# FraPria/proovread

Hardware: AMD Instinct MI355X
Metric: corrected long-read Mbases/sec per node (higher is better)
Workload: dtype int32

## Files before the change

proovread_amd/csrc/seed_core.h:

```cpp
#pragma once
#include <math.h>
#include <stdint.h>

#include "../../include/prgpu.h"

#if defined(__HIPCC__)
#define SC_HD __host__ __device__ inline
#else
#define SC_HD inline
#endif

#if defined(PR_SEED_STATS) && !defined(__HIP_DEVICE_COMPILE__)
extern unsigned long long pr_seed_stat_g[24];
#define SC_STAT(k, v) __atomic_fetch_add(&pr_seed_stat_g[k], (unsigned long long)(v), __ATOMIC_RELAXED)
#else
#define SC_STAT(k, v) ((void)0)
#endif

namespace prgpu {
namespace seedc {

constexpr int KI = 12;
constexpr uint32_t NK = 1u << (2 * KI);
constexpr int KX = 28;
constexpr uint64_t KX_MASK = (1ull << (2 * KX)) - 1;
#ifndef SC_SCANGE
#define SC_SCANGE 1
#endif
constexpr int HB = 20;
constexpr int CB_SHIFT = 12;
constexpr int RK = 11;

constexpr uint64_t POS_PAGE = 1ull << 32;
constexpr int64_t MAX_TEXT = (int64_t)1 << 33;

struct BlkFr {
    int64_t d0, d1;
    int32_t c0, bnd, bnd2, pad;
};

struct IndexView {
    const uint8_t *text;
    int64_t n_text;
    const int64_t *cstart;
    int32_t n_contig;
    const int32_t *cblk;
    const int64_t *lr_off;
    int32_t n_lr;
    int64_t l_pac;
    const uint64_t *koff;
    const uint32_t *kpos;
    const uint64_t *ksplit;
    const uint64_t *kext;
    const uint32_t *cnt[KI - 1];
    const uint64_t *text4;
    const BlkFr *blkfr;
    int32_t walk_nw = 4;
};

struct Iv {
    int32_t start, end;
    int64_t occ;
};
struct Seed {
    int64_t rbeg;
    int16_t qbeg, len;
    int32_t nx;
};
struct RangeRec {
    int32_t head, tail, n, l_idx;
    int64_t tpos;
    int64_t f_rbeg, l_rbeg;
    int32_t f_ql, l_ql;
    int32_t pad[4];
};
struct RangeEnt {
    int32_t key, r;
};
struct Chain {
    int64_t pos;
    int32_t rid, head, tail, n;
    int32_t w, kept, first;
};

enum {
    SC_OVER_LEN = 1, SC_OVER_HITS = 2, SC_OVER_IV = 4, SC_OVER_MEMS = 8, SC_OVER_SEEDS = 16,
    SC_OVER_CHAINS = 32, SC_OVER_OUT = 64
};

struct Scratch {
    int32_t lmax;
    int32_t *hoff;
    uint64_t *qext;
    int32_t *codes;
    uint32_t *ge;
    uint32_t *hpos;
    uint8_t *hhi;
    uint16_t *hml;
    int32_t cap_hits;
    Iv *mems;
    int32_t cap_mems;
    Iv *m1, *curr, *prev;
    int32_t cap_iv;
    Seed *seeds;
    int32_t cap_seeds;
    Chain *cv, *ch;
    int32_t *cnx, *kept;
    RangeEnt *htab;
    RangeRec *rg;
    int32_t cap_chains, hsize;
    uint16_t *rmax;
    uint64_t *hfr;
    int32_t *hend;
    uint8_t *ready;
    uint64_t *q4w;
    int32_t *lz;
    int32_t lim_hits;
    bool htab_clean;
};

SC_HD uint64_t pack_ext(const uint8_t *s, int n) {
    uint64_t v = 0;
    int k = 0;
    for (; k < n && s[k] < 4; ++k) v |= (uint64_t)s[k] << (2 * k);
    return v | ((uint64_t)k << 56);
}

SC_HD int ctz64(uint64_t x) { return __builtin_ctzll(x); }

SC_HD uint8_t base_code(uint8_t c) {
    if (c < 4) return c;
    switch (c | 0x20) {
        case 'a': return 0;
        case 'c': return 1;
        case 'g': return 2;
        case 't': return 3;
        default: return 4;
    }
}

SC_HD uint64_t hit_pos(const IndexView &I, uint32_t code, uint64_t r) {
    uint64_t p = I.kpos[r];
    if (I.ksplit && r >= I.ksplit[code]) p += POS_PAGE;
    return p;
}
SC_HD uint64_t get_hpos(const Scratch &S, int64_t k) {
    return (uint64_t)S.hpos[k] | (S.hhi ? (uint64_t)S.hhi[k] << 32 : 0ull);
}
SC_HD void set_hpos(const Scratch &S, int64_t k, uint64_t p) {
    if (!S.hpos) return;
    S.hpos[k] = (uint32_t)p;
    if (S.hhi) S.hhi[k] = (uint8_t)(p >> 32);
}

SC_HD int contig_of(const IndexView &I, int64_t p) {
    int c = I.cblk[p >> CB_SHIFT];
    while (c + 1 < I.n_contig && I.cstart[c + 1] <= p) ++c;
    return c;
}

SC_HD void text_to_fr(const IndexView &I, uint64_t p, int64_t &fr, int &rid) {
    const int c = contig_of(I, p);
    const int64_t o = (int64_t)p - I.cstart[c];
    if (c < I.n_lr) {
        rid = c;
        fr = I.lr_off[c] + o;
// ... 567 lines not shown
        if constexpr (occ_lazy<OccT>::value) return S.lz[1] != 0;
        else return false;
    };
    auto push = [&](const Iv &v) {
        if (nm >= S.cap_mems) {
            err |= SC_OVER_MEMS;
            return;
        }
        S.mems[nm++] = v;
    };
    for (int x = 0; x < len && !err && !over();) {
        if (q[x] < 4) {
            x = smem1(occ, S, q, len, x, 1, S.m1, n1, err);
            for (int k = 0; k < n1; ++k)
                if (S.m1[k].end - S.m1[k].start >= O.min_seed_len) push(S.m1[k]);
        } else {
            ++x;
        }
    }
    SC_TICK(0);
    const int split_len = (int)(O.min_seed_len * O.split_factor + .499);
    const int nfirst = nm;
    for (int k = 0; k < nfirst && !err && !over(); ++k) {
        const Iv p = S.mems[k];
        if (p.end - p.start < split_len || p.occ > O.split_width) continue;
        smem1(occ, S, q, len, (p.start + p.end) >> 1, p.occ + 1, S.m1, n1, err);
        for (int j = 0; j < n1; ++j)
            if (S.m1[j].end - S.m1[j].start >= O.min_seed_len) push(S.m1[j]);
    }
    SC_TICK(1);
    if (O.max_mem_intv > 0) {
        for (int x = 0; x < len && !err && !over();) {
            if (q[x] < 4) {
                Iv m;
                x = seed_strategy1(occ, q, len, x, O.min_seed_len, O.max_mem_intv, m);
                if (m.occ > 0) push(m);
            } else {
                ++x;
            }
        }
    }
    if (over()) return nm;
    if (nm > 1 && S.cap_seeds >= nm && !err && !S.hend) {
        static_assert(sizeof(Seed) == sizeof(Iv), "the seed pool holds the sorted intervals");
        int32_t *cnt = S.codes;
        Iv *tmp = reinterpret_cast<Iv *>(S.seeds);
        for (int x = 0; x <= len; ++x) cnt[x] = 0;
        for (int i = 0; i < nm; ++i) ++cnt[S.mems[i].start + 1];
        for (int x = 1; x <= len; ++x) cnt[x] += cnt[x - 1];
        for (int i = 0; i < nm; ++i) {
            const Iv v = S.mems[i];
            tmp[cnt[v.start]++] = v;
        }
        for (int i = 0; i < nm; ++i) {
            const Iv v = tmp[i];
            int j = i - 1;
            while (j >= 0 && S.mems[j].start == v.start && S.mems[j].end > v.end) {
                S.mems[j + 1] = S.mems[j];
                --j;
            }
            S.mems[j + 1] = v;
        }
    } else {
        for (int i = 1; i < nm; ++i) {
            const Iv v = S.mems[i];
            int j = i - 1;
            while (j >= 0 && (S.mems[j].start > v.start || (S.mems[j].start == v.start && S.mems[j].end > v.end))) {
                S.mems[j + 1] = S.mems[j];
                --j;
            }
            S.mems[j + 1] = v;
        }
    }
    SC_TICK(2);
    return nm;
}

SC_HD int range_slot(const Scratch &S, int32_t key) {
    uint32_t h = ((uint32_t)key * 0x9E3779B1u) & (uint32_t)(S.hsize - 1);
    while (S.htab[h].key != -1 && S.htab[h].key != key) h = (h + 1) & (uint32_t)(S.hsize - 1);
    return (int)h;
}
SC_HD int32_t pack_ql(const Seed &s) { return (int32_t)(uint16_t)s.qbeg | ((int32_t)s.len << 16); }

SC_HD int test_and_merge(const pr_seed_opts &O, int64_t l_pac, Scratch &S, int32_t &ns, Chain &c, const Seed &p,
                         int rid) {
    const Seed &last = S.seeds[c.tail];
    const Seed &first = S.seeds[c.head];
    const int64_t qend = last.qbeg + last.len, rend = last.rbeg + last.len;
    if (rid != c.rid) return 0;
    if (p.qbeg >= first.qbeg && p.qbeg + p.len <= qend && p.rbeg >= first.rbeg && p.rbeg + p.len <= rend)
        return 1;
    if ((last.rbeg < l_pac || first.rbeg < l_pac) && p.rbeg >= l_pac) return 0;
    const int64_t x = p.qbeg - last.qbeg, y = p.rbeg - last.rbeg;
    if (y >= 0 && x - y <= O.w && y - x <= O.w && x - last.len < O.max_chain_gap && y - last.len < O.max_chain_gap) {
        if (ns >= S.cap_seeds) return -1;
        S.seeds[ns] = p;
        S.seeds[ns].nx = -1;
        S.seeds[c.tail].nx = ns;
        c.tail = ns++;
        ++c.n;
        return 1;
    }
    return 0;
}

SC_HD int merge_tail(const pr_seed_opts &O, int64_t l_pac, Scratch &S, int32_t &ns, RangeRec &R, const Seed &p) {
    const int64_t f_rbeg = R.f_rbeg, l_rbeg = R.l_rbeg;
    const int f_q = (int16_t)(R.f_ql & 0xFFFF), l_q = (int16_t)(R.l_ql & 0xFFFF), l_len = R.l_ql >> 16;
    const int64_t qend = l_q + l_len, rend = l_rbeg + l_len;
    if (p.qbeg >= f_q && p.qbeg + p.len <= qend && p.rbeg >= f_rbeg && p.rbeg + p.len <= rend)
        return 1;
    if ((l_rbeg < l_pac || f_rbeg < l_pac) && p.rbeg >= l_pac) return 0;
    const int64_t x = p.qbeg - l_q, y = p.rbeg - l_rbeg;
    if (y >= 0 && x - y <= O.w && y - x <= O.w && x - l_len < O.max_chain_gap && y - l_len < O.max_chain_gap) {
        if (ns >= S.cap_seeds) return -1;
        S.seeds[ns] = p;
        S.seeds[ns].nx = -1;
        S.seeds[R.l_idx].nx = ns;
        R.l_idx = ns++;
        R.l_rbeg = p.rbeg;
        R.l_ql = pack_ql(p);
        ++R.n;
        return 1;
    }
    return 0;
}
SC_HD void flush_tail(Scratch &S, const RangeRec &R) {
    S.cv[R.tail].tail = R.l_idx;
    S.cv[R.tail].n = R.n;
}

SC_HD int chain_weight(const Scratch &S, const Chain &c) {
    int64_t qe = 0, re = 0;
    int wq = 0, wr = 0;
    for (int32_t k = c.head; k >= 0;) {
        const Seed s = S.seeds[k];
        if (s.qbeg >= qe) wq += s.len;
        else if (s.qbeg + s.len > qe) wq += (int)(s.qbeg + s.len - qe);
        qe = qe > s.qbeg + s.len ? qe : s.qbeg + s.len;
        if (s.rbeg >= re) wr += s.len;
        else if (s.rbeg + s.len > re) wr += (int)(s.rbeg + s.len - re);
        re = re > s.rbeg + s.len ? re : s.rbeg + s.len;
        k = s.nx;
    }
    const int w = wr < wq ? wr : wq;
    return w < (1 << 30) ? w : (1 << 30) - 1;
}

SC_HD int cal_max_gap(const pr_seed_opts &O, int qlen) {
    int l_del = (int)((double)(qlen * O.a - O.o_del) / O.e_del + 1.);
    int l_ins = (int)((double)(qlen * O.a - O.o_ins) / O.e_ins + 1.);
    int l = l_del > l_ins ? l_del : l_ins;
    l = l > 1 ? l : 1;
    return l < O.w << 1 ? l : O.w << 1;
}

SC_HD int seed_flt_min_score(const pr_seed_opts &O, int len) {
    double min_l;
    if (O.min_chain_weight) min_l = (double)(1.1f * (float)O.min_chain_weight);
    else min_l = (double)5.5f * log((double)len);
    if (min_l > (double)(0.05f * (float)len)) return -1;
    return (int)(O.a * min_l + .499);
}

template <class T>
SC_HD int seed_sw_score(const IndexView &I, const pr_seed_opts &O, const uint8_t *q, int len, const Seed &s, int rid,
                        T *H, T *E, int stride = 1) {
    if (s.len >= 200) return -1;
    int qb = s.qbeg - 50, qe = s.qbeg + s.len + 50;
    qb = qb > 0 ? qb : 0;
    qe = qe < len ? qe : len;
    int64_t rb = s.rbeg - 50, re = s.rbeg + s.len + 50;
    const int64_t mid = (s.rbeg + s.rbeg + s.len) >> 1;
    rb = rb > 0 ? rb : 0;
    re = re < (I.l_pac << 1) ? re : (I.l_pac << 1);
    if (rb < I.l_pac && I.l_pac < re) {
        if (mid < I.l_pac) re = I.l_pac;
        else rb = I.l_pac;
    }
    if (qe - qb >= 200 || re - rb >= 200) return -1;
    const bool rev = mid >= I.l_pac;
    const int64_t fb = rev ? (I.l_pac << 1) - I.lr_off[rid + 1] : I.lr_off[rid];
    const int64_t fe = rev ? (I.l_pac << 1) - I.lr_off[rid] : I.lr_off[rid + 1];
    rb = rb > fb ? rb : fb;
    re = re < fe ? re : fe;
    const int64_t tc = rev ? I.cstart[2 * I.n_lr - 1 - rid] : I.cstart[rid];
    const uint8_t *t = I.text + tc + (rb - fb);
    const int qn = qe - qb, tn = (int)(re - rb);
    const int oe_del = O.o_del + O.e_del, oe_ins = O.o_ins + O.e_ins;
    for (int j = 0; j < qn; ++j) H[j * stride] = 0, E[j * stride] = 0;
    int best = 0;
    for (int i = 0; i < tn; ++i) {
        const int ti = t[i];
        int hdiag = 0, f = 0;
        for (int j = 0; j < qn; ++j) {
            const int qj = q[qb + j];
            const int sc = (ti > 3 || qj > 3) ? -1 : (ti == qj ? O.a : -O.b);
            int h = hdiag + sc;
            const int e = E[j * stride];
            h = h > e ? h : e;
            h = h > f ? h : f;
            h = h > 0 ? h : 0;
            hdiag = H[j * stride];
            H[j * stride] = (T)h;
            best = best > h ? best : h;
            int en = e - O.e_del, eo = h - oe_del;
            en = en > eo ? en : eo;
            E[j * stride] = (T)(en > 0 ? en : 0);
            int fn = f - O.e_ins, fo = h - oe_ins;
            fn = fn > fo ? fn : fo;
            f = fn > 0 ? fn : 0;
        }
    }
    return best;
}

SC_HD void chain_flt(const pr_seed_opts &O, Scratch &S, int ncv, int *n_chains);
template <bool LZ = false>
SC_HD int chain_seq(const IndexView &I, const pr_seed_opts &O, Scratch &S, int nm, int *n_cv);

template <bool LZ = false>
SC_HD int map_chains(const IndexView &I, const pr_seed_opts &O, Scratch &S, const uint8_t *q, int len, int *n_chains,
                     unsigned long long *ticks = nullptr, const uint32_t *lcnt = nullptr) {
    *n_chains = 0;
    int err = 0;
#if defined(__HIP_DEVICE_COMPILE__)
    unsigned long long t_last = ticks ? __builtin_amdgcn_s_memrealtime() : 0ULL;
#endif
    const OccB<LZ> occ{&I, &S, q, len, lcnt};
    const int nm = collect_intv(occ, S, O, q, len, err, ticks);
    if (LZ) err |= S.lz[1];
    if (err) return err;
    SC_STAT(0, 1);
    SC_STAT(1, nm);
#if defined(__HIP_DEVICE_COMPILE__)
    if (ticks) t_last = __builtin_amdgcn_s_memrealtime();
#endif
    int ncv = 0;
    err = chain_seq<LZ>(I, O, S, nm, &ncv);
    if (LZ) err |= S.lz[1];
    if (err) return err;
    SC_TICK(3);
    SC_STAT(11, ncv);
    SC_STAT(12, (unsigned long long)ncv * ncv);
    chain_flt(O, S, ncv, n_chains);
    SC_TICK(4);
    return 0;
}

template <bool LZ>
SC_HD int chain_seq(const IndexView &I, const pr_seed_opts &O, Scratch &S, int nm, int *n_cv) {
    const bool clean_on_entry = S.htab_clean;
    int32_t ns = 0, ncv = 0, nrg = 0;
    if (!clean_on_entry)
        for (int k = 0; k < S.hsize; ++k) S.htab[k].key = -1;
    auto leave = [&](int rc) {
        if (clean_on_entry)
            for (int r = 0; r < nrg; ++r) S.htab[S.rg[r].pad[0]].key = -1;
        return rc;
    };
    for (int mi = 0; mi < nm; ++mi) {
        const Iv p = S.mems[mi];
        const int slen = p.end - p.start;
        if (LZ && !S.ready[p.start]) return leave(SC_OVER_HITS);
        const int32_t h0 = S.hoff[p.start], h1 = LZ ? S.hend[p.start] : S.hoff[p.start + 1];
        const int64_t np = p.occ;
        const int64_t step = np > O.max_occ ? np / O.max_occ : 1;
        int64_t fidx = 0, take = 0, count = 0;
        constexpr int CB = 8;
        int32_t k = h0;
        while (k < h1 && count < O.max_occ) {
            int32_t sel[CB];
            int nsel = 0;
            while (k < h1 && count < O.max_occ && nsel < CB) {
                uint16_t ml[8];
#pragma unroll
                for (int u = 0; u < 8; ++u) ml[u] = k + u < h1 ? S.hml[k + u] : (uint16_t)0;
                int u = 0;
                for (; u < 8 && k < h1 && count < O.max_occ && nsel < CB; ++u, ++k) {
                    if (ml[u] < slen) continue;
                    const bool use = fidx == take;
                    ++fidx;
                    if (!use) continue;
                    take += step;
                    ++count;
                    sel[nsel++] = k;
                }
            }
            int64_t rb[CB];
            int rd[CB], hsl[CB];
            int32_t key[CB];
#pragma unroll
            for (int u = 0; u < CB; ++u) {
                const uint64_t v = u < nsel ? S.hfr[sel[u]] : 0ull;
                rb[u] = (int64_t)(v >> FR_RID_BITS);
                rd[u] = (int)(v & ((1u << FR_RID_BITS) - 1u));
                key[u] = rd[u] * 2 + (rb[u] >= I.l_pac ? 1 : 0);
            }
#pragma unroll
            for (int u = 0; u < CB; ++u) hsl[u] = u < nsel ? range_slot(S, key[u]) : 0;
            bool opened = false;
            for (int u = 0; u < nsel; ++u) {
                SC_STAT(3, 1);
                Seed s;
                s.rbeg = rb[u];
                s.qbeg = (int16_t)p.start;
                s.len = (int16_t)slen;
                s.nx = -1;
                const int rid = rd[u];
                const int hs = opened ? range_slot(S, key[u]) : hsl[u];
                const RangeEnt e = S.htab[hs];
                const bool found = e.key == key[u];
                int at = -1;
                bool at_tail = false;
                if (found) {
                    RangeRec &R = S.rg[e.r];
                    SC_STAT(4, 1);
                    if (R.tpos <= s.rbeg) {
                        at = R.tail;
                        at_tail = true;
                    } else {
                        for (int x = R.head; x >= 0 && S.cv[x].pos <= s.rbeg; x = S.cnx[x]) {
                            at = x;
                            SC_STAT(4, 1);
                        }
                    }
                    if (at >= 0) {
                        const int r = at_tail ? merge_tail(O, I.l_pac, S, ns, R, s)
                                              : test_and_merge(O, I.l_pac, S, ns, S.cv[at], s, rid);
                        if (r < 0) return leave(SC_OVER_SEEDS);
                        if (r) { SC_STAT(5, 1); continue; }
                    }
                }
                SC_STAT(6, 1);
                if (ncv >= S.cap_chains) return leave(SC_OVER_CHAINS);
                if (ns >= S.cap_seeds) return leave(SC_OVER_SEEDS);
                S.seeds[ns] = s;
                Chain c;
                c.pos = s.rbeg;
                c.rid = rid;
                c.head = c.tail = ns;
                c.n = 1;
                c.w = c.kept = 0;
                c.first = -1;
                S.cv[ncv] = c;
                if (!found) {
                    RangeRec &R = S.rg[nrg];
                    R.head = R.tail = ncv;
                    R.n = 1;
                    R.l_idx = ns;
                    R.tpos = s.rbeg;
                    R.f_rbeg = R.l_rbeg = s.rbeg;
                    R.f_ql = R.l_ql = pack_ql(s);
                    R.pad[0] = hs;
                    S.htab[hs].key = key[u];
                    S.htab[hs].r = nrg++;
                    S.cnx[ncv] = -1;
                    opened = true;
                } else {
                    RangeRec &R = S.rg[e.r];
                    if (at < 0) {
                        S.cnx[ncv] = R.head;
                        R.head = ncv;
                    } else {
                        const int nx = S.cnx[at];
                        S.cnx[ncv] = nx;
                        S.cnx[at] = ncv;
                        if (nx < 0) {
                            flush_tail(S, R);
                            R.tail = ncv;
                            R.n = 1;
                            R.l_idx = ns;
                            R.tpos = s.rbeg;
                            R.f_rbeg = R.l_rbeg = s.rbeg;
                            R.f_ql = R.l_ql = pack_ql(s);
                        }
                    }
                }
                ++ns;
                ++ncv;
            }
        }
    }
    for (int r = 0; r < nrg; ++r) {
        flush_tail(S, S.rg[r]);
        if (clean_on_entry) S.htab[S.rg[r].pad[0]].key = -1;
    }
    *n_cv = ncv;
    return 0;
}

SC_HD void chain_flt(const pr_seed_opts &O, Scratch &S, int ncv, int *n_chains) {
    int nch = 0;
    const bool keep_all = O.drop_ratio <= 0;
    for (int j = 0; j < ncv; ++j) {
        Chain c = S.cv[j];
        c.w = chain_weight(S, c);
        if (keep_all) c.kept = 3;
        if (c.w >= O.min_chain_weight) S.ch[nch++] = c;
    }
    for (int i = 1; i < nch; ++i) {
        const Chain v = S.ch[i];
        int j = i - 1;
        while (j >= 0 && (S.ch[j].w < v.w || (S.ch[j].w == v.w && (S.ch[j].pos > v.pos ||
                                                                   (S.ch[j].pos == v.pos && S.ch[j].head > v.head))))) {
            S.ch[j + 1] = S.ch[j];
            --j;
            SC_STAT(13, 1);
        }
        S.ch[j + 1] = v;
    }
    if (nch > 0 && !keep_all) {
        int nk = 1;
        S.kept[0] = 0;
        S.ch[0].kept = 3;
        for (int i = 1; i < nch; ++i) {
            int large = 0, k;
            const int bi = S.seeds[S.ch[i].head].qbeg;
            const int ei = S.seeds[S.ch[i].tail].qbeg + S.seeds[S.ch[i].tail].len;
            for (k = 0; k < nk; ++k) {
                Chain &cj = S.ch[S.kept[k]];
                const int bj = S.seeds[cj.head].qbeg;
                const int ej = S.seeds[cj.tail].qbeg + S.seeds[cj.tail].len;
                const int bmax = bj > bi ? bj : bi;
                const int emin = ej < ei ? ej : ei;
                if (emin > bmax) {
                    const int li = ei - bi, lj = ej - bj;
                    const int minl = li < lj ? li : lj;
                    if (emin - bmax >= minl * O.mask_level && minl < O.max_chain_gap) {
                        large = 1;
                        if (cj.first < 0) cj.first = i;
                        if (S.ch[i].w < cj.w * O.drop_ratio && cj.w - S.ch[i].w >= O.min_seed_len << 1) break;
                    }
                }
            }
            if (k == nk) {
                S.kept[nk++] = i;
                S.ch[i].kept = large ? 2 : 3;
            }
        }
        for (int k = 0; k < nk; ++k)
            if (S.ch[S.kept[k]].first >= 0) S.ch[S.ch[S.kept[k]].first].kept = 1;
    }
    *n_chains = nch;
}

SC_HD int flt_seed_list(const Scratch &S, int nch, int32_t *list, int cap) {
    int n = 0;
    for (int ci = 0; ci < nch; ++ci) {
        const Chain &c = S.ch[ci];
        if (c.kept == 0) continue;
        for (int32_t k = c.head; k >= 0; k = S.seeds[k].nx) {
            if (n >= cap) return -1;
            list[n++] = k;
        }
    }
    return n;
}

SC_HD int map_output(const IndexView &I, const pr_seed_opts &O, Scratch &S, const uint8_t *q, int len, int sid,
                     int nch, pr_seed_task *out, int cap_out, int *n_out, const int32_t *scores = nullptr,
                     unsigned long long *ticks = nullptr, int16_t *dp16 = nullptr) {
    *n_out = 0;
#if defined(__HIP_DEVICE_COMPILE__)
    unsigned long long t_last = ticks ? __builtin_amdgcn_s_memrealtime() : 0ULL;
#endif
    const int flt = seed_flt_min_score(O, len);
    int32_t *swH = (int32_t *)S.ge, *swE = swH + 201;
    int no = 0, nkept = 0;
    for (int ci = 0; ci < nch; ++ci) {
        const Chain &c = S.ch[ci];
        if (c.kept == 0) continue;
        const bool rev = S.seeds[c.head].rbeg >= I.l_pac;
        const int64_t L = I.lr_off[c.rid + 1] - I.lr_off[c.rid];
        const int64_t cs = rev ? I.l_pac + (I.l_pac - I.lr_off[c.rid + 1]) : I.lr_off[c.rid];
        if (no + c.n > cap_out) return SC_OVER_OUT;
        const int first = no;
        int idx = 0;
        int64_t r0 = INT64_MAX, r1 = INT64_MIN;
        for (int32_t k = c.head; k >= 0; k = S.seeds[k].nx) {
            const Seed &s = S.seeds[k];
            int score = s.len;
            if (flt >= 0) {
                const int x = scores ? scores[k]
                                     : (dp16 ? seed_sw_score(I, O, q, len, s, c.rid, dp16, dp16 + 201 * 64, 64)
                                             : seed_sw_score(I, O, q, len, s, c.rid, swH, swE));
                if (x >= 0 && x < flt) continue;
                score = x < 0 ? s.len * O.a : x;
            }
            const int64_t b = s.rbeg - (s.qbeg + cal_max_gap(O, s.qbeg));
            const int64_t e = s.rbeg + s.len + ((len - s.qbeg - s.len) + cal_max_gap(O, len - s.qbeg - s.len));
            r0 = r0 < b ? r0 : b;
            r1 = r1 > e ? r1 : e;
            pr_seed_task &t = out[no];
            t.sr = sid;
            t.lr = c.rid;
            t.strand = rev ? 1 : 0;
            t.qbeg = s.qbeg;
            t.rbeg = (int32_t)(s.rbeg - cs);
            t.slen = s.len;
            t.chain = nkept;
            t.rmax0 = score;
            t.rank = idx++;
            int j = no - 1;
            while (j >= first && (out[j].rmax0 < t.rmax0 || (out[j].rmax0 == t.rmax0 && out[j].rank < t.rank))) --j;
            const pr_seed_task v = t;
            for (int m = no; m > j + 1; --m) out[m] = out[m - 1];
            out[j + 1] = v;
            ++no;
        }
        if (no == first) continue;
        r0 -= cs;
        r1 -= cs;
        for (int m = first; m < no; ++m) {
            out[m].rank = m - first;
            out[m].rmax0 = (int32_t)(r0 > 0 ? r0 : 0);
            out[m].rmax1 = (int32_t)(r1 < L ? r1 : L);
        }
        ++nkept;
    }
    *n_out = no;
// ... 162 lines not shown
```

proovread_amd/csrc/seed_kernels.hip:

```cpp
#include <hip/hip_runtime.h>

#include <rocprim/device/device_radix_sort.hpp>

#include "seed_core.h"
#include "seed_dev.h"

namespace prgpu {

#ifndef SEED_WAVES_DEF
#define SEED_WAVES_DEF 4
#endif
#ifndef SEED_LMAX_DEF
#define SEED_LMAX_DEF 1024
#endif
constexpr int SEED_WAVES = SEED_WAVES_DEF;
constexpr int SEED_LMAX = SEED_LMAX_DEF;
#ifndef SEED_MINB
#define SEED_MINB 4
#endif
#ifndef SEED_WAVE_MINB
#define SEED_WAVE_MINB SEED_MINB
#endif
#ifndef OCC_U
#define OCC_U 2
// ... 247 lines not shown
                        bool go = a + ml < len;
                        constexpr int nw = NW;
                        while (go) {
                            const uint64_t tp = p[u] + (uint64_t)ml;
                            const uint64_t* tw4 = V.text4 + (tp >> 4);
                            const int sh = (int)(tp & 15) * 4;
                            uint64_t w5[5];
#pragma unroll
                            for (int j = 0; j < 5; ++j) w5[j] = j <= nw ? tw4[j] : 0ull;
#pragma unroll
                            for (int j = 0; j < 4; ++j) {
                                if (!go || j >= nw) break;
                                const int x = a + ml;
                                const uint64_t tw = sh ? (w5[j] >> sh) | (w5[j + 1] << (64 - sh)) : w5[j];
                                const uint64_t qw = nib16(q4, (uint64_t)x);
                                const uint64_t nq = (qw >> 2) & 0x1111111111111111ull;
                                const uint64_t bad = (qw ^ tw) | (nq * 0xFull);
                                const int lim = len - x;
                                if (bad) {
                                    const int f = __builtin_ctzll(bad) >> 2;
                                    ml += f < lim ? f : lim;
                                    go = false;
                                } else if (lim <= 16) {
                                    ml += lim;
                                    go = false;
                                } else {
                                    ml += 16;
                                }
                            }
                        }
                    } else {
                        while (a + ml < len && q[a + ml] < 4 && V.text[p[u] + ml] == q[a + ml]) ++ml;
                    }
                }
                seedc::set_hpos(S, k, p[u]);
                const int64_t fr = (int64_t)p[u] + dlt[u];
                const int rid = c[u] < V.n_lr ? c[u] : 2 * V.n_lr - 1 - c[u];
                S.hfr[k] = ((uint64_t)fr << seedc::FR_RID_BITS) | (uint64_t)rid;
                S.hml[k] = (uint16_t)(ml < 65535 ? ml : 65535);
            }
        }
        __threadfence_block();
        wave_sync_lds();
        OCC_TICK(1);
        const seedc::Occ occ{&V, &S, q, len, lc};
        for (int a = lane; a < len; a += 64) {
            uint32_t g[HB];
            uint16_t top[seedc::RK];
#pragma unroll
            for (int t = 0; t < HB; ++t) g[t] = 0u;
#pragma unroll
            for (int k = 0; k < seedc::RK; ++k) top[k] = 0;
            const bool has = a + KI <= len && S.codes[a] >= 0;
            const bool ranked = has && q[a] < 4;
            if (has) {
                const int h0 = ho[a], h1 = ho[a + 1];
                for (int h = h0; h < h1; h += 4) {
                    uint64_t w4;
                    __builtin_memcpy(&w4, S.hml + h, 8);
#pragma unroll
                    for (int j = 0; j < 4; ++j) {
                        if (h + j >= h1) break;
                        const uint16_t ml = (uint16_t)(w4 >> (16 * j));
                        const int d = (int)ml - KI;
#pragma unroll
                        for (int t = 0; t < HB; ++t) g[t] += d >= t ? 1u : 0u;
                        if (ranked) seedc::topk_insert(top, ml);
                    }
                }
            }
            uint32_t *dst = S.ge + (int64_t)a * HB;
#pragma unroll
            for (int t = 0; t < HB; ++t) dst[t] = g[t];
            seedc::fill_rk_top(occ, S, q, len, a, top);
        }
        __threadfence_block();
    }
    wave_sync_lds();
    OCC_TICK(2);
#undef OCC_TICK
    return err;
}

__device__ int chain_wave(const seedc::IndexView &I, const pr_seed_opts &O, seedc::Scratch &S, int nm, int lane,
                          int32_t *lds) {
    using namespace seedc;
    int2 *ol = reinterpret_cast<int2 *>(S.ge);
    const int cap_ge = (int)((int64_t)S.lmax * HB * 4 / 12);
    const int cap2 = 2 * S.cap_chains;
    const int cap = cap_ge < S.cap_seeds ? (cap_ge < cap2 ? cap_ge : cap2) : (S.cap_seeds < cap2 ? S.cap_seeds : cap2);
    const unsigned long long below = (1ull << lane) - 1ull;
    int n = 0;
    wave_sync_lds();
    for (int mi = 0; mi < nm && n >= 0; ++mi) {
        const Iv p = S.mems[mi];
        const int slen = p.end - p.start;
        const int32_t h0 = S.hoff[p.start], h1 = S.hoff[p.start + 1];
        const int step = p.occ > O.max_occ ? (int)(p.occ / O.max_occ) : 1;
        int fbase = 0, count = 0;
        for (int32_t kb = h0; kb < h1 && count < O.max_occ; kb += 64) {
            const int32_t k = kb + lane;
            const bool qual = k < h1 && S.hml[k] >= slen;
            const unsigned long long qm = __ballot(qual);
            const int f = fbase + __popcll(qm & below);
            const bool use = qual && f % step == 0 && f / step < O.max_occ;
            const unsigned long long um = __ballot(use);
            const int nu = __popcll(um);
            if (n + nu > cap) {
                n = -1;
                break;
            }
            if (use) ol[n + __popcll(um & below)] = make_int2(k, mi);
            n += nu;
            count += nu;
            fbase += __popcll(qm);
        }
    }
    if (n < 0) return -1;
    int32_t *idx = reinterpret_cast<int32_t *>(ol + n);
    int32_t *cnt = lds, *cur = lds + 64;
    cnt[lane] = 0;
    for (int e = lane; e < n; e += 64) S.cv[e].n = 0;
    for (int k = lane; k < S.hsize; k += 64) S.htab[k].key = -1;
    if (lane == 0) lds[128] = 0;
    __threadfence_block();
    wave_sync_lds();
    auto owner_of = [&](int e) -> int {
        const uint64_t v = S.hfr[ol[e].x];
        const int rid = (int)(v & ((1u << FR_RID_BITS) - 1u));
        const int key = rid * 2 + ((int64_t)(v >> FR_RID_BITS) >= I.l_pac ? 1 : 0);
        return (int)(((uint32_t)key * 0x9E3779B1u) >> 26);
    };
    for (int pass = 0; pass < 2; ++pass) {
        if (pass == 1) {
            int x = cnt[lane];
#pragma unroll
            for (int d = 1; d < 64; d <<= 1) {
                const int y = __shfl_up(x, d, 64);
                if (lane >= d) x += y;
            }
            cur[lane] = x - cnt[lane];
            wave_sync_lds();
        }
        for (int e0 = 0; e0 < n; e0 += 64) {
            const int e = e0 + lane;
            const int own = e < n ? owner_of(e) : 64;
            unsigned long long m = __ballot(e < n);
#pragma unroll
            for (int b = 0; b < 7; ++b) {
                const bool bit = (own >> b) & 1;
                const unsigned long long w = __ballot(bit);
                m &= bit ? w : ~w;
            }
            const int rank = __popcll(m & below);
            const bool leader = e < n && rank == 0;
            if (pass == 0) {
                if (leader) atomicAdd(&cnt[own], __popcll(m));
            } else {
                if (e < n) idx[cur[own] + rank] = e;
                wave_sync_lds();
                if (leader) cur[own] += __popcll(m);
            }
            wave_sync_lds();
        }
        wave_sync_lds();
    }
    __threadfence_block();
    wave_sync_lds();
    const int mine = cnt[lane], first = cur[lane] - mine;
    for (int t = 0; t < mine; ++t) {
        const int e = idx[first + t];
        const int2 oe = ol[e];
        const Iv p = S.mems[oe.y];
        const uint64_t v = S.hfr[oe.x];
        Seed sd;
        sd.rbeg = (int64_t)(v >> FR_RID_BITS);
        sd.qbeg = (int16_t)p.start;
        sd.len = (int16_t)(p.end - p.start);
        sd.nx = -1;
        const int rid = (int)(v & ((1u << FR_RID_BITS) - 1u));
        const int32_t key = rid * 2 + (sd.rbeg >= I.l_pac ? 1 : 0);
        uint32_t h = ((uint32_t)key * 0x9E3779B1u) & (uint32_t)(S.hsize - 1);
        bool found = false;
        for (;;) {
            const int32_t kk = S.htab[h].key;
            if (kk == key) { found = true; break; }
            if (kk == -1) {
                const int32_t old = atomicCAS(&S.htab[h].key, -1, key);
                if (old == -1) break;
                if (old == key) { found = true; break; }
            }
            h = (h + 1) & (uint32_t)(S.hsize - 1);
        }
        int at = -1;
        bool at_tail = false;
        int32_t ns = e;
        if (found && S.htab[h].r < 0) continue;
        if (found) {
            RangeRec &R = S.rg[S.htab[h].r];
            if (R.tpos <= sd.rbeg) {
                at = R.tail;
                at_tail = true;
            } else {
                for (int x = R.head; x >= 0 && S.cv[x].pos <= sd.rbeg; x = S.cnx[x]) at = x;
            }
            if (at >= 0) {
                const int r = at_tail ? merge_tail(O, I.l_pac, S, ns, R, sd)
                                      : test_and_merge(O, I.l_pac, S, ns, S.cv[at], sd, rid);
                if (r) continue;
            }
        }
        S.seeds[e] = sd;
        Chain c;
        c.pos = sd.rbeg;
        c.rid = rid;
        c.head = c.tail = e;
        c.n = 1;
        c.w = c.kept = 0;
        c.first = -1;
        S.cv[e] = c;
        if (!found) {
            const int r = atomicAdd(&lds[128], 1);
            if (r >= S.cap_chains) {
                S.htab[h].r = -1;
                continue;
            }
            RangeRec &R = S.rg[r];
            R.head = R.tail = e;
            R.n = 1;
            R.l_idx = e;
            R.tpos = sd.rbeg;
            R.f_rbeg = R.l_rbeg = sd.rbeg;
            R.f_ql = R.l_ql = pack_ql(sd);
            S.htab[h].r = r;
            S.cnx[e] = -1;
        } else {
            RangeRec &R = S.rg[S.htab[h].r];
            if (at < 0) {
                S.cnx[e] = R.head;
                R.head = e;
            } else {
                const int nx = S.cnx[at];
                S.cnx[e] = nx;
                S.cnx[at] = e;
                if (nx < 0) {
                    flush_tail(S, R);
                    R.tail = e;
                    R.n = 1;
                    R.l_idx = e;
                    R.tpos = sd.rbeg;
                    R.f_rbeg = R.l_rbeg = sd.rbeg;
                    R.f_ql = R.l_ql = pack_ql(sd);
                }
            }
        }
    }
    __threadfence_block();
    wave_sync_lds();
    const int nrg = lds[128];
    if (nrg > S.cap_chains) return -2;
    for (int r = lane; r < nrg; r += 64) flush_tail(S, S.rg[r]);
    __threadfence_block();
    wave_sync_lds();
    int ncv = 0;
    for (int e0 = 0; e0 < n; e0 += 64) {
        const int e = e0 + lane;
        Chain c{};
        if (e < n) c = S.cv[e];
        const bool live = e < n && c.n > 0;
        const unsigned long long lm = __ballot(live);
        wave_sync_lds();
        if (live) S.cv[ncv + __popcll(lm & below)] = c;
        ncv += __popcll(lm);
        __threadfence_block();
        wave_sync_lds();
    }
    return ncv > S.cap_chains ? -2 : ncv;
}

__device__ bool chain_flt_wave(const pr_seed_opts &O, seedc::Scratch &S, int ncv, int lane, int *n_chains) {
    using namespace seedc;
    const int64_t ge_bytes = (int64_t)S.lmax * HB * 4;
    if ((int64_t)ncv * 36 > ge_bytes) return false;
    struct Key { int32_t nw, head; int64_t pos; };
    const bool keep_all = O.drop_ratio <= 0;
    Key *key = reinterpret_cast<Key *>(S.ge);
    for (int j = lane; j < ncv; j += 64) {
        Chain &c = S.cv[j];
        const int w = chain_weight(S, c);
        c.w = w;
        key[j] = Key{w >= O.min_chain_weight ? -w : INT32_MAX, c.head, c.pos};
    }
    __threadfence_block();
    wave_sync_lds();
    int nch = 0;
    for (int ib = 0; ib < ncv; ib += 64) {
        const int i = ib + lane;
        const Key ki = i < ncv ? key[i] : Key{INT32_MAX, 0, 0};
        const bool pass = ki.nw != INT32_MAX;
        nch += __popcll(__ballot(pass));
        int rank = 0;
        for (int jb = 0; jb < ncv; jb += 64) {
            const Key kj = jb + lane < ncv ? key[jb + lane] : Key{INT32_MAX, 0, 0};
            const int plo = (int)(uint32_t)kj.pos, phi = (int)(kj.pos >> 32);
#pragma unroll
            for (int t = 0; t < 64; ++t) {
                const int nw = __builtin_amdgcn_readlane(kj.nw, t), hd = __builtin_amdgcn_readlane(kj.head, t);
                const int64_t ps = (int64_t)(((uint64_t)(uint32_t)__builtin_amdgcn_readlane(phi, t) << 32) |
                                             (uint32_t)__builtin_amdgcn_readlane(plo, t));
                rank += (nw < ki.nw || (nw == ki.nw && (ps < ki.pos || (ps == ki.pos && hd < ki.head)))) ? 1 : 0;
            }
        }
        if (pass) {
            Chain c = S.cv[i];
            if (keep_all) c.kept = 3;
            S.ch[rank] = c;
        }
    }
    __threadfence_block();
    wave_sync_lds();
    if (keep_all) {
        *n_chains = nch;
        return true;
    }
    int4 *iv = reinterpret_cast<int4 *>(S.ge);
    int4 *kv = iv + nch;
    int32_t *fm = reinterpret_cast<int32_t *>(kv + nch);
    for (int i = lane; i < nch; i += 64) {
        const Chain &c = S.ch[i];
        const Seed &h = S.seeds[c.head], &t = S.seeds[c.tail];
        iv[i] = make_int4(h.qbeg, t.qbeg + t.len, c.w, 0);
        fm[i] = -1;
    }
    __threadfence_block();
    wave_sync_lds();
    if (nch > 0) {
        int nk = 1;
        if (lane == 0) {
            kv[0] = iv[0];
            S.ch[0].kept = 3;
        }
        __threadfence_block();
        wave_sync_lds();
        for (int i = 1; i < nch; ++i) {
            const int4 ci = iv[i];
            const int bi = ci.x, ei = ci.y;
            bool large = false, drop = false;
            for (int kb = 0; kb < nk && !drop; kb += 64) {
                const int k = kb + lane;
                bool ov = false, br = false;
                if (k < nk) {
                    const int4 cj = kv[k];
                    const int bj = cj.x, ej = cj.y;
                    const int bmax = bj > bi ? bj : bi;
                    const int emin = ej < ei ? ej : ei;
                    if (emin > bmax) {
                        const int li = ei - bi, lj = ej - bj;
                        const int minl = li < lj ? li : lj;
                        if (emin - bmax >= minl * O.mask_level && minl < O.max_chain_gap) {
                            ov = true;
                            br = ci.z < cj.z * O.drop_ratio && cj.z - ci.z >= O.min_seed_len << 1;
                        }
                    }
                }
                const unsigned long long bm = __ballot(br);
                const int last = bm ? __ffsll((long long)bm) - 1 : 63;
                if (ov && lane <= last && fm[k] < 0) fm[k] = i;
                large = large || __ballot(ov && lane <= last) != 0ull;
                drop = bm != 0ull;
            }
            if (!drop) {
                if (lane == 0) {
                    kv[nk] = ci;
                    S.ch[i].kept = large ? 2 : 3;
                }
                ++nk;
                __threadfence_block();
                wave_sync_lds();
            }
        }
        __threadfence_block();
        wave_sync_lds();
        for (int k = lane; k < nk; k += 64)
            if (fm[k] >= 0) S.ch[fm[k]].kept = 1;
    }
    __threadfence_block();
    wave_sync_lds();
    *n_chains = nch;
    return true;
}

template <int NW>
__global__ void __launch_bounds__(64 * SEED_WAVES, SEED_WAVE_MINB) seed_wave_kernel(SeedDev D) {
    __shared__ __attribute__((aligned(16))) int32_t hoff_lds[SEED_WAVES][SEED_LMAX + 4];
    __shared__ uint64_t q4_lds[SEED_WAVES][SEED_LMAX / 16 + 4];
    __shared__ uint32_t lcnt[seedc::LC_N];
    load_lcnt(D.V, lcnt);
    const int lane = threadIdx.x & 63, wv = threadIdx.x >> 6;
    const int64_t slot = (int64_t)blockIdx.x * SEED_WAVES + wv;
    if (slot >= D.n_lanes) return;
    seedc::Scratch S = seedc::carve(D.scratch + slot * D.stride, D.caps);
    int32_t *ho = hoff_lds[wv];
    unsigned long long pt[4] = {0ULL, 0ULL, 0ULL, 0ULL};
    unsigned long long pl[6] = {0ULL, 0ULL, 0ULL, 0ULL, 0ULL, 0ULL};
    for (;;) {
        int j = 0;
        if (lane == 0) j = atomicAdd(D.next, 1);
        j = __shfl(j, 0, 64);
        if (j >= D.n_list) {
            if (D.prof && lane == 0) {
                pt[1] += pl[0] + pl[1] + pl[2];
                pt[2] += pl[3] + pl[4];
                pt[3] += pl[5];
                for (int k = 0; k < 4; ++k) atomicAdd(&D.prof[k], pt[k]);
            }
            break;
        }
        const int i = D.rlist ? D.rlist[j] : j;
        const int64_t o = D.sr_off[i];
        const int len = (int)(D.sr_off[i + 1] - o);
        const uint8_t *q = D.sr_seq + o;
        int err = 0;
        const unsigned long long t0 = D.prof && lane == 0 ? wall_clock64() : 0ULL;
        if (len > S.lmax || len > SEED_LMAX - 1) err = seedc::SC_OVER_LEN;
        if (len > 0 && !err) err = build_occ_wave<NW>(D.V, S, q, len, ho, lane, q4_lds[wv], lcnt);
        int nch = 0, nlist = -1, nm = 0;
        unsigned long long tm = 0ULL;
        if (lane == 0) {
            if (D.prof) {
                tm = wall_clock64();
                pt[0] += tm - t0;
                atomicMax(&D.prof[17], tm - t0);
            }
            if (len > 0 && !err) {
                const seedc::Occ occ{&D.V, &S, q, len, lcnt};
                nm = seedc::collect_intv(occ, S, D.O, q, len, err, D.prof ? pl : nullptr);
            }
            if (D.prof) atomicMax(&D.prof[18], wall_clock64() - tm);
        }
        err = __shfl(err, 0, 64);
        nm = __shfl(nm, 0, 64);
        if (len > 0 && !err) {
            const unsigned long long tc = D.prof && lane == 0 ? wall_clock64() : 0ULL;
            __threadfence_block();
            int ncv = chain_wave(D.V, D.O, S, nm, lane, ho);
            unsigned long long tf = D.prof && lane == 0 ? wall_clock64() : 0ULL;
            if (lane == 0 && D.prof) atomicAdd(&D.prof[14 + (ncv == -1 ? 1 : 0)], tf - tc);
            if (ncv == -2) {
                ncv = 0;
                err = seedc::SC_OVER_CHAINS;
            }
            if (lane == 0 && ncv == -1) {
                ncv = 0;
                err = seedc::chain_seq(D.V, D.O, S, nm, &ncv);
                if (D.prof) {
                    const unsigned long long t_ = wall_clock64();
                    atomicAdd(&D.prof[13], 1ULL);
                    atomicAdd(&D.prof[15], t_ - tf);
                    tf = t_;
                }
            }
            err = __shfl(err, 0, 64);
            ncv = __shfl(ncv, 0, 64);
            __threadfence_block();
            wave_sync_lds();
            bool flt = err != 0 || chain_flt_wave(D.O, S, ncv, lane, &nch);
            if (lane == 0) {
                if (!flt) seedc::chain_flt(D.O, S, ncv, &nch);
                if (D.prof) {
                    const unsigned long long t_ = wall_clock64();
                    pl[3] += t_ - tc;
                    atomicAdd(&D.prof[16], t_ - tf);
                }
                if (!err && seedc::seed_flt_min_score(D.O, len) >= 0 && 3 * S.cap_seeds <= 2 * S.cap_hits &&
                    2 * 201 * 64 * 2 <= 4 * S.lmax * seedc::HB)
                    nlist = seedc::flt_seed_list(S, nch, (int32_t *)S.hfr + S.cap_seeds, S.cap_seeds);
            }
        }
        err = __shfl(err, 0, 64);
        nlist = __shfl(nlist, 0, 64);
        if (nlist > 0) {
            __threadfence_block();
            const int32_t *list = (const int32_t *)S.hfr + S.cap_seeds;
            int32_t *rid = (int32_t *)S.hfr + 2 * S.cap_seeds;
            if (lane == 0) {
                int x = 0;
                for (int ci = 0; ci < nch; ++ci) {
                    const seedc::Chain &c = S.ch[ci];
                    if (c.kept == 0) continue;
                    for (int32_t k = c.head; k >= 0; k = S.seeds[k].nx) rid[x++] = c.rid;
                }
            }
            __threadfence_block();
            int32_t *scores = (int32_t *)S.hfr;
            int16_t *H = (int16_t *)S.ge + lane, *E = H + 201 * 64;
            for (int x = lane; x < nlist; x += 64) {
                const int32_t k = list[x];
                scores[k] = seedc::seed_sw_score(D.V, D.O, q, len, S.seeds[k], rid[x], H, E, 64);
            }
            __threadfence_block();
        }
        if (lane == 0) {
            int n = 0;
            if (len > 0 && !err)
                err = seedc::map_output(D.V, D.O, S, q, len, i, nch, D.out + (int64_t)(i - D.out0) * D.caps.out,
                                        D.caps.out, &n, nlist >= 0 ? (const int32_t *)S.hfr : nullptr,
                                        D.prof ? pl : nullptr);
            D.n_out[i] = err ? 0 : n;
            D.status[i] = err;
            if (D.prof) atomicMax(&D.prof[19], wall_clock64() - t0);
        }
        __threadfence_block();
    }
}

template <bool LZ>
__global__ void __launch_bounds__(64 * SEED_WAVES, SEED_MINB) seed_batch_kernel(SeedDev D) {
    __shared__ __attribute__((aligned(16))) int32_t hoff_lds[SEED_WAVES][SEED_LMAX + 4];
    __shared__ uint64_t q4_lds[SEED_WAVES][SEED_LMAX / 16 + 4];
    __shared__ uint32_t lcnt[seedc::LC_N];
    load_lcnt(D.V, lcnt);
    const int lane = threadIdx.x & 63, wv = threadIdx.x >> 6;
    const int64_t slot = (int64_t)blockIdx.x * SEED_WAVES + wv;
    if (slot >= D.n_lanes) return;
    int batch = 64;
    if constexpr (LZ) batch = D.batch;
    uint8_t *base = D.scratch + slot * batch * D.stride;
    int32_t *ho = hoff_lds[wv];
    unsigned long long pt[2] = {0ULL, 0ULL};
    unsigned long long lt[6] = {0ULL, 0ULL, 0ULL, 0ULL, 0ULL, 0ULL};
    unsigned long long ot[3] = {0ULL, 0ULL, 0ULL};
    constexpr bool HTAB_REUSE = LZ;
    if (HTAB_REUSE) {
        struct __attribute__((aligned(8))) Ent2 { seedc::RangeEnt a, b; };
        const seedc::Scratch S0 = seedc::carve(base, D.caps);
        const int64_t off = reinterpret_cast<uint8_t *>(S0.htab) - base;
        const Ent2 free2{{-1, -1}, {-1, -1}};
        for (int rd = 0; rd < batch; ++rd) {
            Ent2 *t = reinterpret_cast<Ent2 *>(base + (int64_t)rd * D.stride + off);
            for (int k = lane; k < S0.hsize / 2; k += 64) t[k] = free2;
        }
        __threadfence_block();
        wave_sync_lds();
    }
    for (;;) {
        int b0 = 0;
        if (lane == 0) b0 = atomicAdd(D.next, batch);
        b0 = __shfl(b0, 0, 64);
        const int64_t nlim = D.rlist ? D.n_list : D.n_sr;
        if (b0 >= nlim) {
            if (D.prof) {
// ... 196 lines not shown
```

Before: 231.5.

## Track chain weight and query span incrementally during chaining

Chains now carry a compact running state (query coverage, reference coverage, query interval) that is updated on every seed merge. This replaces the later linked-list walk in chain_weight and the head/tail seed lookups in the filter. The sequential filter also gains a compact kept-record array in scratch so overlap checks read contiguous small records instead of full Chain structs. In exchange the Chain struct grows, and weights are clamped to 16 bits, which could diverge from the exact computation for very long chains.

```diff
diff --git a/proovread_amd/csrc/seed_core.h b/proovread_amd/csrc/seed_core.h
--- a/proovread_amd/csrc/seed_core.h
+++ b/proovread_amd/csrc/seed_core.h
@@ -26,6 +26,9 @@
 constexpr uint64_t KX_MASK = (1ull << (2 * KX)) - 1;
 #ifndef SC_SCANGE
 #define SC_SCANGE 1
+#endif
+#ifndef SC_KEPT_COPIES
+#define SC_KEPT_COPIES 1
 #endif
 constexpr int HB = 20;
 constexpr int CB_SHIFT = 12;
@@ -81,7 +84,50 @@
     int64_t pos;
     int32_t rid, head, tail, n;
     int32_t w, kept, first;
+    int32_t qi;
 };
+
+static_assert(sizeof(Chain) == 40 && sizeof(RangeRec) == 64, "scratch slice layout");
+
+struct ChainState {
+    int32_t qc;
+    uint32_t re;
+    int32_t wr;
+};
+SC_HD ChainState chain_state_first(int qbeg, int len) {
+    return ChainState{len | ((qbeg + len) << 16), (uint32_t)len, len};
+}
+SC_HD void chain_state_add(ChainState &st, int qbeg, int len, int64_t rel) {
+    int wq = st.qc & 0xFFFF, qe = (int)((uint32_t)st.qc >> 16);
+    if (qbeg >= qe) wq += len;
+    else if (qbeg + len > qe) wq += qbeg + len - qe;
+    qe = qe > qbeg + len ? qe : qbeg + len;
+    st.qc = wq | (qe << 16);
+    const int64_t re = (int64_t)st.re;
+    int64_t wr = st.wr;
+    if (rel >= re) wr += len;
+    else if (rel + len > re) wr += rel + len - re;
+    st.re = (uint32_t)(re > rel + len ? re : rel + len);
+    st.wr = (int32_t)(wr < 65535 ? wr : 65535);
+}
+SC_HD int chain_state_weight(const ChainState &st) {
+    const int wq = st.qc & 0xFFFF;
+    return st.wr < wq ? st.wr : wq;
+}
+SC_HD void chain_state_put(Chain &c, const ChainState &st, int32_t qi) {
+    c.w = st.qc;
+    c.kept = st.wr;
+    c.first = (int32_t)st.re;
+    c.qi = qi;
+}
+SC_HD ChainState chain_state_get(const Chain &c) { return ChainState{c.w, (uint32_t)c.first, c.kept}; }
+SC_HD int chain_state_settle(Chain &c) {
+    const int w = chain_state_weight(chain_state_get(c));
+    c.w = w;
+    c.kept = 0;
+    c.first = -1;
+    return w;
+}
 
 enum {
     SC_OVER_LEN = 1, SC_OVER_HITS = 2, SC_OVER_IV = 4, SC_OVER_MEMS = 8, SC_OVER_SEEDS = 16,
@@ -815,12 +861,47 @@
     return (int)h;
 }
 SC_HD int32_t pack_ql(const Seed &s) { return (int32_t)(uint16_t)s.qbeg | ((int32_t)s.len << 16); }
-
+SC_HD int32_t pack_qi(int f_qbeg, int l_qend) { return (int32_t)(uint16_t)f_qbeg | (l_qend << 16); }
+
+
+template <bool CS>
+SC_HD Chain chain_open(const Seed &s, int rid, int32_t si) {
+    Chain c;
+    c.pos = s.rbeg;
+    c.rid = rid;
+    c.head = c.tail = si;
+    c.n = 1;
+    if constexpr (CS) {
+        chain_state_put(c, chain_state_first(s.qbeg, s.len), pack_qi(s.qbeg, s.qbeg + s.len));
+    } else {
+        c.w = c.kept = 0;
+        c.first = -1;
+    }
+    return c;
+}
+template <bool CS>
+SC_HD void tail_open(RangeRec &R, int32_t ci, int32_t si, const Seed &s) {
+    R.tail = ci;
+    R.n = 1;
+    R.l_idx = si;
+    R.tpos = s.rbeg;
+    R.f_rbeg = R.l_rbeg = s.rbeg;
+    R.f_ql = R.l_ql = pack_ql(s);
+    if constexpr (CS) {
+        const ChainState st = chain_state_first(s.qbeg, s.len);
+        R.pad[1] = st.qc;
+        R.pad[2] = (int32_t)st.re;
+        R.pad[3] = st.wr;
+    }
+}
+
+template <bool CS>
 SC_HD int test_and_merge(const pr_seed_opts &O, int64_t l_pac, Scratch &S, int32_t &ns, Chain &c, const Seed &p,
                          int rid) {
     const Seed &last = S.seeds[c.tail];
     const Seed &first = S.seeds[c.head];
     const int64_t qend = last.qbeg + last.len, rend = last.rbeg + last.len;
+    const int f_q = first.qbeg;
     if (rid != c.rid) return 0;
     if (p.qbeg >= first.qbeg && p.qbeg + p.len <= qend && p.rbeg >= first.rbeg && p.rbeg + p.len <= rend)
         return 1;
@@ -833,11 +914,18 @@
         S.seeds[c.tail].nx = ns;
         c.tail = ns++;
         ++c.n;
+        if constexpr (CS) {
+            ChainState st = chain_state_get(c);
+            chain_state_add(st, p.qbeg, p.len, p.rbeg - c.pos);
+            chain_state_put(c, st, pack_qi(f_q, p.qbeg + p.len));
+        }
+        SC_STAT(18, 1);
         return 1;
     }
     return 0;
 }
 
+template <bool CS>
 SC_HD int merge_tail(const pr_seed_opts &O, int64_t l_pac, Scratch &S, int32_t &ns, RangeRec &R, const Seed &p) {
     const int64_t f_rbeg = R.f_rbeg, l_rbeg = R.l_rbeg;
     const int f_q = (int16_t)(R.f_ql & 0xFFFF), l_q = (int16_t)(R.l_ql & 0xFFFF), l_len = R.l_ql >> 16;
@@ -855,13 +943,27 @@
         R.l_rbeg = p.rbeg;
         R.l_ql = pack_ql(p);
         ++R.n;
+        if constexpr (CS) {
+            ChainState st{R.pad[1], (uint32_t)R.pad[2], R.pad[3]};
+            chain_state_add(st, p.qbeg, p.len, p.rbeg - R.tpos);
+            R.pad[1] = st.qc;
+            R.pad[2] = (int32_t)st.re;
+            R.pad[3] = st.wr;
+        }
         return 1;
     }
     return 0;
 }
+template <bool CS>
 SC_HD void flush_tail(Scratch &S, const RangeRec &R) {
-    S.cv[R.tail].tail = R.l_idx;
-    S.cv[R.tail].n = R.n;
+    Chain &c = S.cv[R.tail];
+    c.tail = R.l_idx;
+    c.n = R.n;
+    if constexpr (CS) {
+        const int l_q = (int16_t)(R.l_ql & 0xFFFF), l_len = R.l_ql >> 16;
+        chain_state_put(c, ChainState{R.pad[1], (uint32_t)R.pad[2], R.pad[3]},
+                        pack_qi((int16_t)(R.f_ql & 0xFFFF), l_q + l_len));
+    }
 }
 
 SC_HD int chain_weight(const Scratch &S, const Chain &c) {
@@ -949,8 +1051,9 @@
     return best;
 }
 
+template <bool CS = false>
 SC_HD void chain_flt(const pr_seed_opts &O, Scratch &S, int ncv, int *n_chains);
-template <bool LZ = false>
+template <bool LZ = false, bool CS = LZ>
 SC_HD int chain_seq(const IndexView &I, const pr_seed_opts &O, Scratch &S, int nm, int *n_cv);
 
 template <bool LZ = false>
@@ -977,12 +1080,12 @@
     SC_TICK(3);
     SC_STAT(11, ncv);
     SC_STAT(12, (unsigned long long)ncv * ncv);
-    chain_flt(O, S, ncv, n_chains);
+    chain_flt<LZ>(O, S, ncv, n_chains);
     SC_TICK(4);
     return 0;
 }
 
-template <bool LZ>
+template <bool LZ, bool CS>
 SC_HD int chain_seq(const IndexView &I, const pr_seed_opts &O, Scratch &S, int nm, int *n_cv) {
     const bool clean_on_entry = S.htab_clean;
     int32_t ns = 0, ncv = 0, nrg = 0;
@@ -1060,8 +1163,8 @@
                         }
                     }
                     if (at >= 0) {
-                        const int r = at_tail ? merge_tail(O, I.l_pac, S, ns, R, s)
-                                              : test_and_merge(O, I.l_pac, S, ns, S.cv[at], s, rid);
+                        const int r = at_tail ? merge_tail<CS>(O, I.l_pac, S, ns, R, s)
+                                              : test_and_merge<CS>(O, I.l_pac, S, ns, S.cv[at], s, rid);
                         if (r < 0) return leave(SC_OVER_SEEDS);
                         if (r) { SC_STAT(5, 1); continue; }
                     }
@@ -1070,22 +1173,11 @@
                 if (ncv >= S.cap_chains) return leave(SC_OVER_CHAINS);
                 if (ns >= S.cap_seeds) return leave(SC_OVER_SEEDS);
                 S.seeds[ns] = s;
-                Chain c;
-                c.pos = s.rbeg;
-                c.rid = rid;
-                c.head = c.tail = ns;
-                c.n = 1;
-                c.w = c.kept = 0;
-                c.first = -1;
-                S.cv[ncv] = c;
+                S.cv[ncv] = chain_open<CS>(s, rid, ns);
                 if (!found) {
                     RangeRec &R = S.rg[nrg];
-                    R.head = R.tail = ncv;
-                    R.n = 1;
-                    R.l_idx = ns;
-                    R.tpos = s.rbeg;
-                    R.f_rbeg = R.l_rbeg = s.rbeg;
-                    R.f_ql = R.l_ql = pack_ql(s);
+                    R.head = ncv;
+                    tail_open<CS>(R, ncv, ns, s);
                     R.pad[0] = hs;
                     S.htab[hs].key = key[u];
                     S.htab[hs].r = nrg++;
@@ -1101,13 +1193,8 @@
                         S.cnx[ncv] = nx;
                         S.cnx[at] = ncv;
                         if (nx < 0) {
-                            flush_tail(S, R);
-                            R.tail = ncv;
-                            R.n = 1;
-                            R.l_idx = ns;
-                            R.tpos = s.rbeg;
-                            R.f_rbeg = R.l_rbeg = s.rbeg;
-                            R.f_ql = R.l_ql = pack_ql(s);
+                            flush_tail<CS>(S, R);
+                            tail_open<CS>(R, ncv, ns, s);
                         }
                     }
                 }
@@ -1117,19 +1204,29 @@
         }
     }
     for (int r = 0; r < nrg; ++r) {
-        flush_tail(S, S.rg[r]);
+        flush_tail<CS>(S, S.rg[r]);
         if (clean_on_entry) S.htab[S.rg[r].pad[0]].key = -1;
     }
     *n_cv = ncv;
     return 0;
 }
 
+template <bool CS>
 SC_HD void chain_flt(const pr_seed_opts &O, Scratch &S, int ncv, int *n_chains) {
     int nch = 0;
     const bool keep_all = O.drop_ratio <= 0;
     for (int j = 0; j < ncv; ++j) {
         Chain c = S.cv[j];
-        c.w = chain_weight(S, c);
+        if constexpr (CS) {
+            chain_state_settle(c);
+#if defined(PR_SEED_CHECK) && !defined(__HIP_DEVICE_COMPILE__)
+            if (c.w != chain_weight(S, c) ||
+                c.qi != pack_qi(S.seeds[c.head].qbeg, S.seeds[c.tail].qbeg + S.seeds[c.tail].len))
+                __builtin_trap();
+#endif
+        } else {
+            c.w = chain_weight(S, c);
+        }
         if (keep_all) c.kept = 3;
         if (c.w >= O.min_chain_weight) S.ch[nch++] = c;
     }
@@ -1144,7 +1241,50 @@
         }
         S.ch[j + 1] = v;
     }
-    if (nch > 0 && !keep_all) {
+    struct alignas(8) KeptRec { int32_t qi, w, first, idx; };
+    if (CS && SC_KEPT_COPIES && nch > 0 && !keep_all &&
+        (int64_t)nch * (int64_t)sizeof(KeptRec) <= (int64_t)S.lmax * HB * 4) {
+        KeptRec *kv = reinterpret_cast<KeptRec *>(S.ge);
+        int nk = 1;
+        kv[0] = KeptRec{S.ch[0].qi, S.ch[0].w, -1, 0};
+        S.ch[0].kept = 3;
+        for (int i = 1; i < nch; ++i) {
+            int large = 0, k;
+            const int32_t qi = S.ch[i].qi;
+            const int wi = S.ch[i].w;
+            const int bi = (int16_t)(qi & 0xFFFF), ei = qi >> 16;
+            for (k = 0; k < nk; ++k) {
+                const KeptRec cj = kv[k];
+                const int bj = (int16_t)(cj.qi & 0xFFFF), ej = cj.qi >> 16;
+                const int bmax = bj > bi ? bj : bi;
+                const int emin = ej < ei ? ej : ei;
+                if (emin > bmax) {
+                    const int li = ei - bi, lj = ej - bj;
+                    const int minl = li < lj ? li : lj;
+                    if (emin - bmax >= minl * O.mask_level && minl < O.max_chain_gap) {
+                        large = 1;
+                        if (cj.first < 0) {
+                            kv[k].first = i;
+                            SC_STAT(20, 1);
+                        }
+                        if (wi < cj.w * O.drop_ratio && cj.w - wi >= O.min_seed_len << 1) break;
+                    }
+                }
+            }
+            if (k == nk) {
+                kv[nk++] = KeptRec{qi, wi, -1, i};
+                S.ch[i].kept = large ? 2 : 3;
+            } else {
+                SC_STAT(19, 1);
+            }
+        }
+        for (int k = 0; k < nk; ++k)
+            if (kv[k].first >= 0) {
+                S.ch[kv[k].idx].first = kv[k].first;
+                S.ch[kv[k].first].kept = 1;
+            }
+    } else if (nch > 0 && !keep_all) {
+        if (CS) SC_STAT(21, 1);
         int nk = 1;
         S.kept[0] = 0;
         S.ch[0].kept = 3;
@@ -1163,7 +1303,10 @@
                     const int minl = li < lj ? li : lj;
                     if (emin - bmax >= minl * O.mask_level && minl < O.max_chain_gap) {
                         large = 1;
-                        if (cj.first < 0) cj.first = i;
+                        if (cj.first < 0) {
+                            cj.first = i;
+                            SC_STAT(20, 1);
+                        }
                         if (S.ch[i].w < cj.w * O.drop_ratio && cj.w - S.ch[i].w >= O.min_seed_len << 1) break;
                     }
                 }
@@ -1171,6 +1314,8 @@
             if (k == nk) {
                 S.kept[nk++] = i;
                 S.ch[i].kept = large ? 2 : 3;
+            } else {
+                SC_STAT(19, 1);
             }
         }
         for (int k = 0; k < nk; ++k)
diff --git a/proovread_amd/csrc/seed_kernels.hip b/proovread_amd/csrc/seed_kernels.hip
--- a/proovread_amd/csrc/seed_kernels.hip
+++ b/proovread_amd/csrc/seed_kernels.hip
@@ -353,6 +353,7 @@
     return err;
 }
 
+template <bool CS>
 __device__ int chain_wave(const seedc::IndexView &I, const pr_seed_opts &O, seedc::Scratch &S, int nm, int lane,
                           int32_t *lds) {
     using namespace seedc;
@@ -476,20 +477,13 @@
                 for (int x = R.head; x >= 0 && S.cv[x].pos <= sd.rbeg; x = S.cnx[x]) at = x;
             }
             if (at >= 0) {
-                const int r = at_tail ? merge_tail(O, I.l_pac, S, ns, R, sd)
-                                      : test_and_merge(O, I.l_pac, S, ns, S.cv[at], sd, rid);
+                const int r = at_tail ? merge_tail<CS>(O, I.l_pac, S, ns, R, sd)
+                                      : test_and_merge<CS>(O, I.l_pac, S, ns, S.cv[at], sd, rid);
                 if (r) continue;
             }
         }
         S.seeds[e] = sd;
-        Chain c;
-        c.pos = sd.rbeg;
-        c.rid = rid;
-        c.head = c.tail = e;
-        c.n = 1;
-        c.w = c.kept = 0;
-        c.first = -1;
-        S.cv[e] = c;
+        S.cv[e] = chain_open<CS>(sd, rid, e);
         if (!found) {
             const int r = atomicAdd(&lds[128], 1);
             if (r >= S.cap_chains) {
@@ -497,12 +491,8 @@
                 continue;
             }
             RangeRec &R = S.rg[r];
-            R.head = R.tail = e;
-            R.n = 1;
-            R.l_idx = e;
-            R.tpos = sd.rbeg;
-            R.f_rbeg = R.l_rbeg = sd.rbeg;
-            R.f_ql = R.l_ql = pack_ql(sd);
+            R.head = e;
+            tail_open<CS>(R, e, e, sd);
             S.htab[h].r = r;
             S.cnx[e] = -1;
         } else {
@@ -515,13 +505,8 @@
                 S.cnx[e] = nx;
                 S.cnx[at] = e;
                 if (nx < 0) {
-                    flush_tail(S, R);
-                    R.tail = e;
-                    R.n = 1;
-                    R.l_idx = e;
-                    R.tpos = sd.rbeg;
-                    R.f_rbeg = R.l_rbeg = sd.rbeg;
-                    R.f_ql = R.l_ql = pack_ql(sd);
+                    flush_tail<CS>(S, R);
+                    tail_open<CS>(R, e, e, sd);
                 }
             }
         }
@@ -530,7 +515,7 @@
     wave_sync_lds();
     const int nrg = lds[128];
     if (nrg > S.cap_chains) return -2;
-    for (int r = lane; r < nrg; r += 64) flush_tail(S, S.rg[r]);
+    for (int r = lane; r < nrg; r += 64) flush_tail<CS>(S, S.rg[r]);
     __threadfence_block();
     wave_sync_lds();
     int ncv = 0;
@@ -549,6 +534,7 @@
     return ncv > S.cap_chains ? -2 : ncv;
 }
 
+template <bool CS>
 __device__ bool chain_flt_wave(const pr_seed_opts &O, seedc::Scratch &S, int ncv, int lane, int *n_chains) {
     using namespace seedc;
     const int64_t ge_bytes = (int64_t)S.lmax * HB * 4;
@@ -558,8 +544,13 @@
     Key *key = reinterpret_cast<Key *>(S.ge);
     for (int j = lane; j < ncv; j += 64) {
         Chain &c = S.cv[j];
-        const int w = chain_weight(S, c);
-        c.w = w;
+        int w;
+        if constexpr (CS) {
+            w = chain_state_settle(c);
+        } else {
+            w = chain_weight(S, c);
+            c.w = w;
+        }
         key[j] = Key{w >= O.min_chain_weight ? -w : INT32_MAX, c.head, c.pos};
     }
     __threadfence_block();
@@ -599,8 +590,12 @@
     int32_t *fm = reinterpret_cast<int32_t *>(kv + nch);
     for (int i = lane; i < nch; i += 64) {
         const Chain &c = S.ch[i];
-        const Seed &h = S.seeds[c.head], &t = S.seeds[c.tail];
-        iv[i] = make_int4(h.qbeg, t.qbeg + t.len, c.w, 0);
+        if constexpr (CS) {
+            iv[i] = make_int4((int16_t)(c.qi & 0xFFFF), c.qi >> 16, c.w, 0);
+        } else {
+            const Seed &h = S.seeds[c.head], &t = S.seeds[c.tail];
+            iv[i] = make_int4(h.qbeg, t.qbeg + t.len, c.w, 0);
+        }
         fm[i] = -1;
     }
     __threadfence_block();
@@ -714,7 +709,8 @@
         if (len > 0 && !err) {
             const unsigned long long tc = D.prof && lane == 0 ? wall_clock64() : 0ULL;
             __threadfence_block();
-            int ncv = chain_wave(D.V, D.O, S, nm, lane, ho);
+            const bool cs = D.O.drop_ratio > 0;
+            int ncv = cs ? chain_wave<true>(D.V, D.O, S, nm, lane, ho) : chain_wave<false>(D.V, D.O, S, nm, lane, ho);
             unsigned long long tf = D.prof && lane == 0 ? wall_clock64() : 0ULL;
             if (lane == 0 && D.prof) atomicAdd(&D.prof[14 + (ncv == -1 ? 1 : 0)], tf - tc);
             if (ncv == -2) {
@@ -723,7 +719,8 @@
             }
             if (lane == 0 && ncv == -1) {
                 ncv = 0;
-                err = seedc::chain_seq(D.V, D.O, S, nm, &ncv);
+                err = cs ? seedc::chain_seq<false, true>(D.V, D.O, S, nm, &ncv)
+                         : seedc::chain_seq<false, false>(D.V, D.O, S, nm, &ncv);
                 if (D.prof) {
                     const unsigned long long t_ = wall_clock64();
                     atomicAdd(&D.prof[13], 1ULL);
@@ -735,9 +732,13 @@
             ncv = __shfl(ncv, 0, 64);
             __threadfence_block();
             wave_sync_lds();
-            bool flt = err != 0 || chain_flt_wave(D.O, S, ncv, lane, &nch);
+            bool flt = err != 0 || (cs ? chain_flt_wave<true>(D.O, S, ncv, lane, &nch)
+                                       : chain_flt_wave<false>(D.O, S, ncv, lane, &nch));
             if (lane == 0) {
-                if (!flt) seedc::chain_flt(D.O, S, ncv, &nch);
+                if (!flt) {
+                    if (cs) seedc::chain_flt<true>(D.O, S, ncv, &nch);
+                    else seedc::chain_flt<false>(D.O, S, ncv, &nch);
+                }
                 if (D.prof) {
                     const unsigned long long t_ = wall_clock64();
                     pl[3] += t_ - tc;
```

Measured after the change: 237.6 (median of 6 runs). 1.03x the previous value.
